# jkworldchampion/Video-Depth-Anything

Measured on AMD Instinct MI355X. Metric: frames/sec at 1x32x518x518 fp16, ViT-L, higher is better.
Workload: dtype f16; 1 GPU; vitl fp16 32-frame clip forward, x=randn(1,32,3,518,518), seeded random weights (BASELINE.json configs[2]); parallelism=independent windows x1, world=1

## Files before the change

include/vda.h:

```cpp
#ifndef VDA_H
#define VDA_H
#include <stddef.h>
#include <stdint.h>

#ifdef __cplusplus
extern "C" {
#endif

typedef void* vda_stream_t;

const char* vda_last_error(void);
int vda_abi_version(void);

enum vda_a_mode {
    VDA_A_DENSE = 0,
    VDA_A_CONV3X3 = 1
};

enum vda_epilogue {
    VDA_EPI_BIAS_F16 = 0,
    VDA_EPI_BIAS_GELU_F16 = 1,
    VDA_EPI_BIAS_RELU_F16 = 2,
    VDA_EPI_SCALE_RES_F32 = 3,
    VDA_EPI_RES_F16 = 4,
// ... 122 lines not shown

int vda_readout_concat_f16(const void* tok, void* out, int frames, int P, int D, vda_stream_t stream);
int vda_readout_concat_f32(const float* tok, float* out, int frames, int P, int D, vda_stream_t stream);

int vda_head_out_f16_f32(const void* in, const float* w, float bias, float* out, int rows, int Cpad, vda_stream_t stream);
int vda_head_out_f32_f32(const float* in, const float* w, float bias, float* out, long long rows, int Cpad, vda_stream_t stream);

int vda_depth_tail_f16(const void* in, const void* w2, const float* b2, const float* w3, float b3, float* out,
                       const void* zero_page, int B, int h, int w, int H, int W, int C, vda_stream_t stream);
int vda_depth_tail_set_variant(int v);
const char* vda_depth_tail_last_kernel(void);

int vda_conv3x3_up2_f16(const void* in, const void* w, const float* bias, void* out, int B, int h, int wd, int C, int N, int ldc,
                        vda_stream_t stream);
int vda_conv3x3_up2_set_variant(int v);
int vda_conv_lds_set_variant(int v);

int vda_normalize_u8_f32(const uint8_t* frames, float* out, int n, int H, int W, vda_stream_t stream);
int vda_gather_normalize_u8_f32(const uint8_t* video, const int32_t* idx, float* out, int n, int n_video, int H, int W,
                                vda_stream_t stream);

int vda_gather_resize_normalize_u8_f32(const uint8_t* video, const int32_t* idx, float* out, int n, int n_video, int H0, int W0,
                                       int H, int W, vda_stream_t stream);

int vda_lsq_scale_shift_f32(const float* pred, const float* target, long long n, double* workspace, int nblk, float* scale_shift,
                            vda_stream_t stream);
int vda_stitch_window_f32(const float* win, const float* scale_shift, float* chunk, float* tail, float* ref1, long long px,
                          const float* wts, vda_stream_t stream);
int vda_affine_clamp_f32(const float* in, const float* scale_shift, float* out, long long n, vda_stream_t stream);
int vda_minmax_accum_f32(const float* x, long long n, float* minmax, vda_stream_t stream);
// ... 94 lines not shown
```

video_depth_anything_amd/_lib.py:

```python
import ctypes as C
import os

_HERE = os.path.dirname(os.path.abspath(__file__))
LIB_PATH = os.environ.get("VDA_LIB_PATH") or os.path.join(_HERE, "libvda_hip.so")

A_DENSE, A_CONV3X3 = 0, 1
(EPI_BIAS_F16, EPI_BIAS_GELU_F16, EPI_BIAS_RELU_F16, EPI_SCALE_RES_F32, EPI_RES_F16, EPI_GEGLU_F16,
 EPI_PATCH_F32, EPI_CONVT_F16, EPI_BIAS_F32, EPI_SCALE_RES_F32_H, EPI_SCALE_RES_SPLIT, EPI_LN_BIAS_F16, EPI_LN_GELU_F16,
 EPI_CONVT_FOLD_F16) = range(14)


class GemmArgs(C.Structure):
    _fields_ = [
        ("A", C.c_void_p), ("W", C.c_void_p), ("bias", C.c_void_p), ("out", C.c_void_p),
        ("res", C.c_void_p), ("res2", C.c_void_p), ("gamma", C.c_void_p), ("pos", C.c_void_p),
        ("zero_page", C.c_void_p),
        ("M", C.c_int32), ("N", C.c_int32), ("K", C.c_int32),
        ("lda", C.c_int32), ("ldc", C.c_int32),
        ("a_mode", C.c_int32), ("epilogue", C.c_int32), ("relu_in", C.c_int32),
        ("cB", C.c_int32), ("cH", C.c_int32), ("cW", C.c_int32), ("cCin", C.c_int32),
        ("cHo", C.c_int32), ("cWo", C.c_int32), ("cStride", C.c_int32),
        ("P", C.c_int32), ("tK", C.c_int32), ("tH", C.c_int32), ("tW", C.c_int32), ("tCout", C.c_int32),
        ("out2", C.c_void_p), ("stats", C.c_void_p), ("sched", C.c_void_p),
        ("stats_ld", C.c_int32), ("tile_rows", C.c_int32),
# ... 31 lines not shown
    "vda_gemm_row_range": (_i, [C.POINTER(GemmArgs), _i, _i, C.POINTER(GemmArgs)]),
    "vda_gemm_last_kernel": (C.c_char_p, []),
    "vda_gemm_plan": (_i, [C.POINTER(GemmArgs), _i, _i, _i, C.POINTER(GemmPlan)]),
    "vda_gemm_launch_name": (_i, [C.POINTER(GemmLaunch), C.c_char_p, _i]),
    "vda_gemm_built": (_i, [_i, _i, _i, _i, _i, _i]),
    "vda_gemm_reload_tuning": (_i, []),
    "vda_layernorm_f32_f16": (_i, [_vp, _vp, _vp, _vp, _f, _i, _i, _i, _i, _vp, _i, _i, _vp]),
    "vda_layernorm_residual_f32_f16": (_i, [_vp, _vp, _vp, _vp, _vp, _vp, _f, _i, _i, _i, _i, _vp]),
    "vda_layernorm_f32_f32": (_i, [_vp, _vp, _vp, _vp, _f, _i, _i, _i, _i, _vp, _i, _i, _vp]),
    "vda_split_stats_f32": (_i, [_vp, _vp, _vp, _vp, _f, _i, _i, _vp]),
    "vda_split_center_stats_f32": (_i, [_vp, _vp, _vp, _vp, _f, _i, _i, _vp]),
    "vda_ln_stats_finalize": (_i, [_vp, _vp, _f, _i, _i, _vp, _vp]),
    "vda_layernorm_split_f16": (_i, [_vp, _vp, _vp, _vp, _vp, _f, _i, _i, _i, _i, _vp]),
    "vda_fold_ln_weight": (_i, [_vp, _vp, _vp, _vp, _vp, _vp, _vp, _i, _i, _vp]),
    "vda_fold_convt_weight": (_i, [_vp, _vp, _vp, _vp, _vp, _i, _i, _i, _i, _i, _vp]),
    "vda_mlp_fused_supported": (_i, [_i, _i]),
    "vda_mlp_permute_w2_f16": (_i, [_vp, _vp, _i, _i, _vp]),
    "vda_mlp_fused_f16": (_i, [_vp, _vp, _vp, _vp, _vp, _vp, _vp, _vp, _vp, _vp, _vp, _i, _i, _i, _i, _vp]),
    "vda_groupnorm_nhwc_f16": (_i, [_vp, _vp, _vp, _vp, _f, _i, _i, _i, _i, _vp, _i, _vp]),
    "vda_groupnorm_nhwc_f32": (_i, [_vp, _vp, _vp, _vp, _f, _i, _i, _i, _i, _vp, _i, _vp]),
    "vda_attention_f16": (_i, [_vp, _vp, _i, _i, _i, _vp]),
    "vda_attention_f32": (_i, [_vp, _vp, _i, _i, _i, _vp]),
    "vda_attention_set_variant": (_i, [_i]),
    "vda_depth_tail_set_variant": (_i, [_i]),
    "vda_depth_tail_last_kernel": (C.c_char_p, []),
    "vda_conv3x3_up2_set_variant": (_i, [_i]),
    "vda_conv_lds_set_variant": (_i, [_i]),
    "vda_temporal_attention_f16": (_i, [_vp, _vp, _i, _i, _i, _i, _vp]),
    "vda_temporal_attention_f32": (_i, [_vp, _vp, _i, _i, _i, _i, _vp]),
    "vda_temporal_attention_set_variant": (_i, [_i]),
# ... 107 lines not shown
```

video_depth_anything_amd/build.py:

```python
import os
import subprocess
import sys
from concurrent.futures import ThreadPoolExecutor

HERE = os.path.dirname(os.path.abspath(__file__))
CSRC = os.path.join(HERE, "csrc")
OBJ = os.path.join(CSRC, "build")
LIB = os.path.join(HERE, "libvda_hip.so")
HIPCC = os.environ.get("HIPCC", "/opt/rocm/bin/hipcc")
FLAGS = ["--offload-arch=gfx950", "-O3", "-std=c++17", "-fPIC", "-ffp-contract=fast", "-Wno-unused-result",
         "-mllvm", "-amdgpu-mfma-vgpr-form"]
PER_FILE = {"stitch.hip": ["-ffp-contract=off"], "eval.hip": ["-ffp-contract=off"], "tae.hip": ["-ffp-contract=off"],
            "resize.hip": ["-ffp-contract=off"], "pointcloud.hip": ["-ffp-contract=off"], "visualize.hip": ["-ffp-contract=off"],
            "losses.hip": ["-ffp-contract=off"], "resize_u8.hip": ["-ffp-contract=off"]}
PER_PREFIX = {"gemm": ["-fno-slp-vectorize"], "attention.hip": ["-fno-slp-vectorize"], "mlp_fused.hip": ["-fno-slp-vectorize"],
              "gemm8p": ["-mllvm", "-amdgpu-atomic-optimizer-strategy=None"]}


def _sources():
    return sorted(f for f in os.listdir(CSRC) if f.endswith(".hip"))


def _deps_mtime():
    hdrs = [os.path.join(CSRC, f) for f in os.listdir(CSRC) if f.endswith(".h")]
    hdrs.append(os.path.join(HERE, "..", "include", "vda.h"))
    return max(os.path.getmtime(h) for h in hdrs)


def _compile(src):
    obj = os.path.join(OBJ, src[:-4] + ".o")
# ... 48 lines not shown
```

video_depth_anything_amd/csrc/host.hip:

```cpp
#include "vda_common.h"
#include <string.h>
#include <exception>
#include <type_traits>
#include <array>
#include <map>
#include <string>
#include <vector>

namespace {

constexpr int PATCH = 14, POS_GRID = 37, KPATCH = 640, GN_GROUPS = 32, TEMPORAL_HEADS = 8;
constexpr float ENC_LN_EPS = 1e-6f, GN_EPS = 1e-6f, TMP_LN_EPS = 1e-5f;

inline int pad64(int c) { return (c + 63) / 64 * 64; }

#define VDA_TRY(expr)            \
    do {                         \
        const int rc_ = (expr);  \
        if (rc_ != 0) return rc_; \
    } while (0)

#define VDA_HIP(expr)                                                      \
    do {                                                                   \
        const hipError_t e_ = (expr);                                      \
// ... 118 lines not shown
    int dyn_sched = 0;
    int ln_fold = VDA_LN_FOLD_DEFAULT;
    int oc1_fused = 1;
    int head_overlap = 0;
    struct Side {
        hipStream_t stream = nullptr;
        hipEvent_t fork = nullptr, join = nullptr, join2 = nullptr;
    };
    std::map<hipStream_t, Side> sides;
    int enc_split = 1;
    std::map<hipStream_t, Side> lanes;
    std::map<hipStream_t, hipEvent_t> tails;
    int head_lanes = 1;
    int convt_fold = 1;
    bool folded[2] = {false, false};
    int mlp_fused = 0;
    volatile int32_t* ovf_host = nullptr;
};

namespace {

using Spec = std::map<std::string, std::vector<int64_t>>;

void build_spec(const vda_config& c, Spec& s) {
    const int64_t D = c.embed_dim, F = c.features;
    const int64_t oc[4] = {c.out_channels[0], c.out_channels[1], c.out_channels[2], c.out_channels[3]};
    auto put = [&](const std::string& k, std::vector<int64_t> v) { s[k] = std::move(v); };
    const std::string p = "pretrained.";
    put(p + "cls_token", {1, 1, D});
    put(p + "pos_embed", {1, POS_GRID * POS_GRID + 1, D});
// ... 225 lines not shown
        VDA_TRY(mat(k + ".w", (size_t)kk * kk * cp * cp, &d));
        hipLaunchKernelGGL((pack_convt_kernel<T>), dim3(grid_for((size_t)kk * kk * cp * cp)), dim3(256), 0, s, raw(n + ".weight"), d, oc[i], oc[i], kk, cp);
        if (vecs) {
            void* bp = nullptr;
            VDA_TRY(dev_alloc(h, (size_t)kk * kk * cp * sizeof(float), &bp));
            h->vec[k + ".b"] = (float*)bp;
            hipLaunchKernelGGL(expand_convt_bias_kernel, dim3((kk * kk * cp + 255) / 256), dim3(256), 0, s, raw(n + ".bias"), (float*)bp, oc[i], kk * kk, cp);
        }
    }
    VDA_TRY(conv("resize3.w", hd + "resize_layers.3.weight", oc[3], oc[3], ocp[3], ocp[3]));
    VDA_TRY(vecp("resize3.b", hd + "resize_layers.3.bias", oc[3], ocp[3]));
    const std::string sc = hd + "scratch.";
    for (int i = 0; i < 4; ++i)
        VDA_TRY(conv("rn" + std::to_string(i + 1) + ".w", sc + "layer" + std::to_string(i + 1) + "_rn.weight", Fe, oc[i], Fe, ocp[i]));
    if constexpr (std::is_same<T, h16>::value) {
        for (int i = 0; i < 2; ++i) {
            const int kk = i == 0 ? 4 : 2;
            const std::string k = "rn" + std::to_string(i + 1) + ".fold";
            T* d = nullptr;
            VDA_TRY(mat(k + ".w", (size_t)kk * kk * Fe * 9 * ocp[i], &d));
            void* bp = nullptr;
            VDA_TRY(dev_alloc(h, (size_t)kk * kk * 9 * Fe * sizeof(float), &bp));
            h->vec[k + ".b"] = (float*)bp;
            VDA_TRY(vda_fold_convt_weight(raw(hd + "resize_layers." + std::to_string(i) + ".weight"), raw(hd + "resize_layers." + std::to_string(i) + ".bias"),
                                          raw(sc + "layer" + std::to_string(i + 1) + "_rn.weight"), d, (float*)bp, kk, oc[i], oc[i], Fe, ocp[i], s));
        }
    }
    for (int i = 1; i <= 4; ++i) {
        const std::string r = sc + "refinenet" + std::to_string(i) + ".", k = "ref" + std::to_string(i) + ".";
        VDA_TRY(lin(k + "out.w", r + "out_conv.weight", Fe, Fe, Fe, Fe));
// ... 262 lines not shown
        const std::string k = "ref" + std::to_string(i) + ".rcu" + std::to_string(u) + ".";
        return conv3x3(x, k + "c1.w", y, B, H, Wd, Fe, Fe, VDA_EPI_BIAS_RELU_F16, 1, V(k + "c1.b"), true);
    }
    int rcu(int i, int u, const void* x, void* out, int B, int H, int Wd, int Fe, const void* res2 = nullptr, const void* y1 = nullptr) {
        const std::string k = "ref" + std::to_string(i) + ".rcu" + std::to_string(u) + ".";
        const void* y = y1;
        if (y1 == nullptr) {
            void* t = act(sp + "rcu_y", (size_t)B * H * Wd * Fe);
            VDA_TRY(rcu_conv1(i, u, x, t, B, H, Wd, Fe));
            y = t;
        }
        VDA_TRY(conv3x3(y, k + "c2.w", out, B, H, Wd, Fe, Fe, VDA_EPI_RES_F16, 1, V(k + "c2.b"), false, x, res2));
        return 0;
    }
    int fusion(int i, const void* x0, const void* x1, int B, int H, int Wd, int Ho, int Wo, int Fe, const std::string& tag, void** result,
               bool upsample = true, const void* y1 = nullptr) {
        const size_t rows = (size_t)B * H * Wd;
        const void* sm = x0;
        if (x1 != nullptr) {
            void* t = act(sp + "fus_s", rows * Fe);
            VDA_TRY(rcu(i, 1, x1, t, B, H, Wd, Fe, x0, y1));
            sm = t;
        }
        void* r = act(sp + "fus_r", rows * Fe);
        VDA_TRY(rcu(i, 2, sm, r, B, H, Wd, Fe));
        void* c = act(upsample ? sp + "fus_c" : tag, rows * Fe);
        const std::string k = "ref" + std::to_string(i) + ".out.";
        VDA_TRY(dense(r, W(k + "w"), c, VDA_EPI_BIAS_F16, (int)rows, Fe, Fe, V(k + "b")));
        if (!upsample) {
            *result = c;
            return 0;
        }
        void* out = act(tag, (size_t)B * Ho * Wo * Fe);
        VDA_TRY(bilinear(c, out, B, H, Wd, Ho, Wo, Fe));
        *result = out;
        return 0;
    }

    int forward(const float* x, float* depth, int B, int T, int H, int Wd) {
        const vda_config& c = h->cfg;
        const int BT = B * T, ph = H / PATCH, pw = Wd / PATCH;
// ... 302 lines not shown
        void* l4 = act("l4", (size_t)BT * h4 * w4 * ocp[3]);
        VDA_TRY(conv3x3(t3, "resize3.w", l4, BT, ph, pw, ocp[3], ocp[3], VDA_EPI_BIAS_F16, 2, V("resize3.b")));
        void* l4t = nullptr;
        VDA_TRY(temporal(1, l4, B, T, h4 * w4, ocp[3], "l4t", &l4t));
        void* l4r = act("l4r", (size_t)BT * h4 * w4 * Fe);
        VDA_TRY(conv3x3(l4t, "rn4.w", l4r, BT, h4, w4, ocp[3], Fe, VDA_EPI_BIAS_F16, 1, nullptr));
        void *p4 = nullptr, *p4t = nullptr, *p3 = nullptr, *p3t = nullptr, *p2 = nullptr, *p1 = nullptr;
        VDA_TRY(fusion(4, l4r, nullptr, BT, h4, w4, ph, pw, Fe, "p4", &p4));
        VDA_TRY(temporal(2, p4, B, T, P, Fe, "p4t", &p4t));
        if (hlanes) VDA_HIP(hipStreamWaitEvent(s, lane->join, 0));
        VDA_TRY(fusion(3, p4t, l3r, BT, ph, pw, h2, w2, Fe, "p3", &p3, true, hlanes ? y1[3] : nullptr));
        VDA_TRY(temporal(3, p3, B, T, h2 * w2, Fe, "p3t", &p3t));
        if (hlanes) VDA_HIP(hipStreamWaitEvent(s, lane->join2, 0));
        VDA_TRY(fusion(2, p3t, l2r, BT, h2, w2, h1, w1, Fe, "p2", &p2, true, hlanes ? y1[2] : nullptr));
        const bool up_fused = prec == VDA_PREC_F16 && h->oc1_fused != 0 && Fhp <= 128 && Fe % 16 == 0;
        VDA_TRY(fusion(1, p2, l1r, BT, h1, w1, 2 * h1, 2 * w1, Fe, up_fused ? "p1c" : "p1", &p1, !up_fused, hlanes ? y1[1] : nullptr));
        const int hh = 2 * h1, ww = 2 * w1;
        void* o1 = act("o1", (size_t)BT * hh * ww * Fhp);
        if (up_fused) {
            if (!dry) VDA_TRY(vda_conv3x3_up2_f16(p1, W("oc1.w"), V("oc1.b"), o1, BT, h1, w1, Fe, Fhp, Fhp, s));
        } else
            VDA_TRY(conv3x3(p1, "oc1.w", o1, BT, hh, ww, Fe, Fhp, VDA_EPI_BIAS_F16, 1, V("oc1.b")));
        if (prec == VDA_PREC_F16) {
            if (!dry) VDA_TRY(vda_depth_tail_f16(o1, W("oc2.w"), V("oc2.b"), V("oc3.w"), h->oc3_bias, depth, h->zero_page, BT, hh, ww, H, Wd, Fhp, s));
        } else {
            void* up = act("tail_up", (size_t)BT * H * Wd * Fhp);
            VDA_TRY(bilinear(o1, up, BT, hh, ww, H, Wd, Fhp));
            void* c2 = act("tail_c2", (size_t)BT * H * Wd * 32);
            VDA_TRY(conv3x3(up, "oc2.w", c2, BT, H, Wd, Fhp, 32, VDA_EPI_BIAS_RELU_F16, 1, V("oc2.b")));
            if (!dry) VDA_TRY(vda_head_out_f32_f32((const float*)c2, V("oc3.w"), h->oc3_bias, depth, (long long)BT * H * Wd, 32, s));
        }
        if (fold && !dry) {
            hipLaunchKernelGGL(poison_on_overflow_kernel, dim3(256), dim3(256), 0, s, (const int*)ovf, depth, (long long)BT * H * Wd, (volatile int*)h->ovf_host);
            VDA_LAUNCH_CHECK();
        }
// ... 34 lines not shown
    VDA_REQUIRE(T <= h->cfg.num_frames, "vda_forward: T=%d exceeds temporal_max_len=%d", T, h->cfg.num_frames);
    VDA_REQUIRE((long long)B * T * ((H / PATCH) * (W / PATCH) + 1) * 4 * h->cfg.embed_dim < (1ll << 31), "vda_forward: clip too large for 32-bit row offsets (B*T*tokens*4*embed_dim)");
    return 0;
}

int head_lanes_default() {
    static const int v = getenv("VDA_HEAD_LANES") ? atoi(getenv("VDA_HEAD_LANES")) : 1;
    return v != 0;
}

int convt_fold_default() {
    static const int v = getenv("VDA_CONVT_FOLD") ? atoi(getenv("VDA_CONVT_FOLD")) : 1;
    return v != 0;
}

int enc_split_default() {
    static const int v = getenv("VDA_ENC_SPLIT") ? atoi(getenv("VDA_ENC_SPLIT")) : 1;
    return v != 0;
}

}

extern "C" int vda_create(const vda_config* cfg, vda_model** out) {
    VDA_REQUIRE(cfg && out, "vda_create: null argument");
    VDA_REQUIRE(cfg->embed_dim > 0 && cfg->embed_dim % 64 == 0 && cfg->num_heads > 0 && cfg->embed_dim == cfg->num_heads * 64,
                "vda_create: embed_dim=%d must be num_heads=%d x 64 (the attention kernels are built for head dim 64)", cfg->embed_dim, cfg->num_heads);
    VDA_REQUIRE(cfg->depth > 0 && cfg->features > 0 && cfg->features % 64 == 0, "vda_create: depth=%d features=%d (features must be a multiple of 64)", cfg->depth, cfg->features);
    VDA_REQUIRE(cfg->num_frames > 0 && cfg->num_frames <= 32, "vda_create: num_frames=%d must be in 1..32", cfg->num_frames);
    VDA_REQUIRE((cfg->use_clstoken | cfg->use_bn | cfg->pe_rope) >> 1 == 0, "vda_create: use_clstoken / use_bn / pe_rope are 0 or 1");
    for (int i = 0; i < 4; ++i) {
// ... 18 lines not shown
        vda_set_error("vda_create: device allocation failed");
        return 2;
    }
    void* ring = nullptr;
    if (hipHostMalloc(&ring, 64, hipHostMallocDefault) != hipSuccess) {
        for (void* p : h->owned) (void)hipFree(p);
        delete h;
        vda_set_error("vda_create: pinned host allocation failed");
        return 2;
    }
    memset(ring, 0, 64);
    h->ovf_host = (volatile int32_t*)ring;
    h->enc_split = enc_split_default();
    h->head_lanes = head_lanes_default();
    h->convt_fold = convt_fold_default();
    *out = h;
    return 0;
}

extern "C" int vda_destroy(vda_model* h) {
    if (h == nullptr) return 0;
    if (h->ovf_host) (void)hipHostFree((void*)h->ovf_host);
    for (auto& kv : h->tails)
        if (kv.second) (void)hipEventDestroy(kv.second);
    for (auto* m : {&h->sides, &h->lanes})
        for (auto& kv : *m) {
            if (kv.second.fork) (void)hipEventDestroy(kv.second.fork);
            if (kv.second.join) (void)hipEventDestroy(kv.second.join);
            if (kv.second.join2) (void)hipEventDestroy(kv.second.join2);
            if (kv.second.stream) (void)hipStreamDestroy(kv.second.stream);
// ... 146 lines not shown

static int vda_debug_copy_impl(vda_model* h, const char* name, void* dst, int64_t bytes, vda_stream_t stream) {
    VDA_REQUIRE(h && name && dst, "vda_debug_copy: null argument");
    auto it = h->layouts.find(h->last_key);
    VDA_REQUIRE(it != h->layouts.end() && h->ws, "vda_debug_copy: no forward has run");
    auto b = it->second.bufs.find(name);
    VDA_REQUIRE(b != it->second.bufs.end(), "vda_debug_copy: no buffer named %s", name);
    VDA_REQUIRE(bytes > 0 && (size_t)bytes <= b->second.second, "vda_debug_copy: %s holds %lld bytes", name, (long long)b->second.second);
    const int lvl = strcmp(name, "l1") == 0 ? 0 : strcmp(name, "l2") == 0 ? 1 : -1;
    if (lvl >= 0 && h->last_key[4] == VDA_PREC_F16 && h->folded[lvl]) {
        VDA_TRY(require_device(h, "vda_debug_copy"));
        Run r{h, VDA_PREC_F16, false, &it->second, (hipStream_t)stream, (size_t)2};
        const int BT = h->last_key[0] * h->last_key[1], ph = h->last_key[2] / PATCH, pw = h->last_key[3] / PATCH;
        VDA_TRY(r.convt(r.act(lvl == 0 ? "t0" : "t1", 0), lvl, r.act(name, 0), BT, ph, pw, h->ocp[lvl]));
    }
    VDA_HIP(hipMemcpyAsync(dst, (char*)h->ws + b->second.first, (size_t)bytes, hipMemcpyDeviceToDevice, (hipStream_t)stream));
    return 0;
}

extern "C" int vda_set_option(vda_model* h, const char* name, int value) {
    VDA_REQUIRE(h && name, "vda_set_option: null argument");
    if (strcmp(name, "residual_in_ln") == 0) {
        h->residual_in_ln = value;
        h->layouts.clear();
        return 0;
    }
    if (strcmp(name, "profile_min_gflop") == 0) {
        h->prof.min_flops = 1e9 * value;
        return 0;
    }
// ... 10 lines not shown
    if (strcmp(name, "head_overlap") == 0) {
        h->head_overlap = value != 0;
        return 0;
    }
    if (strcmp(name, "enc_split") == 0) {
        h->enc_split = value < 0 ? enc_split_default() : value != 0;
        h->layouts.clear();
        return 0;
    }
    if (strcmp(name, "head_lanes") == 0) {
        h->head_lanes = value < 0 ? head_lanes_default() : value != 0;
        return 0;
    }
    if (strcmp(name, "convt_fold") == 0) {
        h->convt_fold = value < 0 ? convt_fold_default() : value != 0;
        return 0;
    }
    if (strcmp(name, "mlp_fused") == 0) {
        h->mlp_fused = value != 0;
        h->layouts.clear();
        return 0;
    }
    if (strcmp(name, "oc1_fused") == 0) {
        h->oc1_fused = value;
        h->layouts.clear();
        return 0;
    }
    vda_set_error("vda_set_option: unknown option %s", name);
    return 1;
}
// ... 111 lines not shown
```

video_depth_anything_amd/engine.py:

```python
import ctypes
import os
from typing import Dict, List

import torch

from . import _lib, ops
from .config import ENC_LN_EPS, GN_EPS, GN_GROUPS, PATCH, POS_GRID, TEMPORAL_HEADS, TMP_LN_EPS, ModelConfig
from .weights import check_state_dict, temporal_channels

F16, F32 = torch.float16, torch.float32
KPATCH = 640


def _pad(c):
    return ops.pad_to(c, 64)


class Engine:
    def __init__(self, cfg: ModelConfig, device="cuda"):
        if not torch.cuda.is_available():
            raise RuntimeError("video_depth_anything_amd needs an MI355X (HIP device); there is no CPU path")
        self.cfg = cfg
        self.device = torch.device(device)
        self.w: Dict[str, torch.Tensor] = {}
        self.act = F16
        self._packs: Dict[torch.dtype, Dict[str, torch.Tensor]] = {}
        self._buf: Dict[tuple, torch.Tensor] = {}
        self._pos_cache: Dict[tuple, torch.Tensor] = {}
        self.loaded = False
        self.residual_in_ln = False
        self.convt_fold = int(os.environ.get("VDA_CONVT_FOLD", "1")) != 0

    def load_state_dict(self, sd, strict=True):
        check_state_dict(self.cfg, sd, strict)
        self._sd = sd
        self._packs.clear()
        self._pos_cache.clear()
        with torch.cuda.device(self.device):
            self._pos_embed_dev = sd["pretrained.pos_embed"].detach().to(self.device, F32).reshape(-1, self.cfg.embed_dim).contiguous()
            self.w = self._pack(F16)
        self.loaded = True

    def _pack(self, dt):
        if dt in self._packs:
            return self._packs[dt]
        cfg, sd = self.cfg, self._sd
# ... 50 lines not shown
        for i in range(4):
            w[f"rn{i + 1}.w"] = conv(f"{sc}layer{i + 1}_rn.weight", Fe, ocp[i])
        if dt == F16:
            for i in (0, 1):
                w[f"rn{i + 1}.fold.w"], w[f"rn{i + 1}.fold.b"] = ops.fold_convt_weight(
                    f32(f"{h}resize_layers.{i}.weight"), f32(f"{h}resize_layers.{i}.bias"), f32(f"{sc}layer{i + 1}_rn.weight"), ocp[i])
        for i in (1, 2, 3, 4):
            r = f"{sc}refinenet{i}."
            w[f"ref{i}.out.w"], w[f"ref{i}.out.b"] = lin(r + "out_conv.weight"), f32(r + "out_conv.bias")
            for u in (1, 2):
                for c in (1, 2):
                    w[f"ref{i}.rcu{u}.c{c}.w"] = conv(f"{r}resConfUnit{u}.conv{c}.weight")
                    w[f"ref{i}.rcu{u}.c{c}.b"] = f32(f"{r}resConfUnit{u}.conv{c}.bias")
        w["oc1.w"] = conv(sc + "output_conv1.weight", Fhp, Fe)
        w["oc1.b"] = padvec(sc + "output_conv1.bias", Fhp)
        w["oc2.w"] = conv(sc + "output_conv2.0.weight", 32, Fhp)
        w["oc2.b"] = f32(sc + "output_conv2.0.bias")
        w["oc3.w"] = f32(sc + "output_conv2.2.weight").reshape(-1)
        self.oc3_bias = float(sd[sc + "output_conv2.2.bias"].reshape(-1)[0])
        for m, Cc in enumerate(temporal_channels(cfg)):
            t = f"{h}motion_modules.{m}.temporal_transformer."
            k = f"tm{m}."
            w[k + "gn.w"], w[k + "gn.b"] = f32(t + "norm.weight"), f32(t + "norm.bias")
            w[k + "in.w"], w[k + "in.b"] = lin(t + "proj_in.weight"), f32(t + "proj_in.bias")
            w[k + "out.w"], w[k + "out.b"] = lin(t + "proj_out.weight"), f32(t + "proj_out.bias")
            tb = t + "transformer_blocks.0."
            for a in (0, 1):
                ab = f"{tb}attention_blocks.{a}."
                qkv = torch.cat([sd[ab + "to_q.weight"], sd[ab + "to_k.weight"], sd[ab + "to_v.weight"]], dim=0)
                w[f"{k}a{a}.qkv.w"] = ops.pack_linear(qkv.detach().to(dv, F32), dtype=dt)
# ... 79 lines not shown
        ops.layernorm(hs, n, w[k + "ffln.w"], w[k + "ffln.b"], TMP_LN_EPS, rows, Cc)
        gg = self.buf("tm_gg", (rows, 4 * Cc), self.act)
        ops.gemm(n, w[k + "ff1.w"], gg, _lib.EPI_GEGLU_F16, M=rows, N=8 * Cc, K=Cc, ldc=4 * Cc, bias=w[k + "ff1.b"])
        hh = self.buf("tm_hh", (rows, Cc), self.act)
        ops.gemm(gg, w[k + "ff2.w"], hh, _lib.EPI_SCALE_RES_F32_H, M=rows, N=Cc, K=4 * Cc, bias=w[k + "ff2.b"], res=hs)
        out = self.buf(tag, (rows, Cc), self.act)
        ops.gemm(hh, w[k + "out.w"], out, _lib.EPI_RES_F16, M=rows, N=Cc, K=Cc, bias=w[k + "out.b"], res=x)
        return out

    def rcu(self, i, u, x, out, B, H, W, Fe, res2=None):
        w = self.w
        y = self.buf("rcu_y", (B * H * W, Fe), self.act)
        self.conv3x3(x, f"ref{i}.rcu{u}.c1.w", y, B, H, W, Fe, Fe, _lib.EPI_BIAS_RELU_F16, bias=w[f"ref{i}.rcu{u}.c1.b"], relu_in=True)
        self.conv3x3(y, f"ref{i}.rcu{u}.c2.w", out, B, H, W, Fe, Fe, _lib.EPI_RES_F16, bias=w[f"ref{i}.rcu{u}.c2.b"], res=x, res2=res2)

    def fusion(self, i, x0, x1, B, H, W, Ho, Wo, Fe, tag, upsample=True):
        w = self.w
        rows = B * H * W
        s = x0
        if x1 is not None:
            s = self.buf("fus_s", (rows, Fe), self.act)
            self.rcu(i, 1, x1, s, B, H, W, Fe, res2=x0)
        r = self.buf("fus_r", (rows, Fe), self.act)
        self.rcu(i, 2, s, r, B, H, W, Fe)
        c = self.buf("fus_c" if upsample else tag, (rows, Fe), self.act)
        ops.gemm(r, w[f"ref{i}.out.w"], c, _lib.EPI_BIAS_F16, M=rows, N=Fe, K=Fe, bias=w[f"ref{i}.out.b"])
        if not upsample:
            return c
        out = self.buf(tag, (B * Ho * Wo, Fe), self.act)
        ops.bilinear_nhwc(c, out, B, H, W, Ho, Wo, Fe)
        return out

    @torch.no_grad()
    def forward(self, x, taps_out: List[torch.Tensor] = None, stages: dict = None, fp32: bool = False):
        if not self.loaded:
            raise RuntimeError("load_state_dict() first")
        with torch.cuda.device(self.device):
            return self._forward(x, taps_out, stages, fp32)

    def _forward(self, x, taps_out, stages, fp32):
# ... 115 lines not shown
        if fold1:
            convt_fold(1, t1, l2r)
        else:
            self.conv3x3(l2, "rn2.w", l2r, BT, h2, w2, ocp[1], Fe, _lib.EPI_BIAS_F16)
        l3r = self.buf("l3r", (BT * P, Fe), self.act)
        self.conv3x3(l3, "rn3.w", l3r, BT, ph, pw, ocp[2], Fe, _lib.EPI_BIAS_F16)
        l4r = self.buf("l4r", (BT * h4 * w4, Fe), self.act)
        self.conv3x3(l4, "rn4.w", l4r, BT, h4, w4, ocp[3], Fe, _lib.EPI_BIAS_F16)

        p4 = self.fusion(4, l4r, None, BT, h4, w4, ph, pw, Fe, "p4")
        p4 = self.temporal(2, p4, B, T, P, Fe, "p4t")
        p3 = self.fusion(3, p4, l3r, BT, ph, pw, h2, w2, Fe, "p3")
        p3 = self.temporal(3, p3, B, T, h2 * w2, Fe, "p3t")
        p2 = self.fusion(2, p3, l2r, BT, h2, w2, h1, w1, Fe, "p2")
        up_fused = not fp32 and Fhp <= 128
        p1 = self.fusion(1, p2, l1r, BT, h1, w1, 2 * h1, 2 * w1, Fe, "p1c" if up_fused else "p1", upsample=not up_fused)

        hh, ww = 2 * h1, 2 * w1
        o1 = self.buf("o1", (BT * hh * ww, Fhp), self.act)
        if up_fused:
            ops.conv3x3_up2(p1, w["oc1.w"], w["oc1.b"], o1, BT, h1, w1, Fe, Fhp, Fhp)
        else:
            self.conv3x3(p1, "oc1.w", o1, BT, hh, ww, Fe, Fhp, _lib.EPI_BIAS_F16, bias=w["oc1.b"])
        depth = torch.empty(B, T, H, W, dtype=F32, device=self.device)
        if not fp32:
            ops.depth_tail(o1, w["oc2.w"], w["oc2.b"], w["oc3.w"], self.oc3_bias, depth, BT, hh, ww, H, W, Fhp)
        else:
            up = self.buf("tail_up", (BT * H * W, Fhp), F32)
            ops.bilinear_nhwc(o1, up, BT, hh, ww, H, W, Fhp)
            c2 = self.buf("tail_c2", (BT * H * W, 32), F32)
            self.conv3x3(up, "oc2.w", c2, BT, H, W, Fhp, 32, _lib.EPI_BIAS_RELU_F16, bias=w["oc2.b"])
            ops.head_out(c2, w["oc3.w"], self.oc3_bias, depth, BT * H * W, 32)
        if stages is not None:
            if fold0:
                convt(0, t0, l1)
            if fold1:
                convt(1, t1, l2)
            stages.update(layer_1=(l1, h1, w1, ocp[0]), layer_2=(l2, h2, w2, ocp[1]), layer_3=(l3, ph, pw, ocp[2]),
                          layer_4=(l4, h4, w4, ocp[3]), path_4=(p4, ph, pw, Fe), path_3=(p3, h2, w2, Fe),
                          path_2=(p2, h1, w1, Fe))
            stages.update(path_1_half=(p1, h1, w1, Fe)) if up_fused else stages.update(path_1=(p1, hh, ww, Fe))
        return depth
```

video_depth_anything_amd/ops.py:

```python
import ctypes as C

import torch

import os
import sys

from . import _lib
from ._lib import GemmArgs, lib
from ._lib import check as _check

_TRACE = os.environ.get("VDA_TRACE_SYNC") == "1"


def check(rc, what=""):
    _check(rc, what)
    if _TRACE:
        sys.stderr.write(f"[vda] {what} ...")
        sys.stderr.flush()
        torch.cuda.synchronize()
        sys.stderr.write(" ok\n")
        sys.stderr.flush()

F16, F32 = torch.float16, torch.float32

# ... 111 lines not shown


def fold_convt_weight(wt, bt, wr, cin_pad=None):
    _req(wt, F32, "wt"), _req(bt, F32, "bt"), _req(wr, F32, "wr")
    Ci, Cm, k, _ = wt.shape
    Co = wr.shape[0]
    if wr.shape[1] != Cm or bt.numel() != Cm or tuple(wr.shape[2:]) != (3, 3) or wt.shape[3] != k:
        raise ValueError("fold_convt_weight: wt [Ci,Cm,k,k], bt [Cm], wr [Co,Cm,3,3]")
    cin_pad = Ci if cin_pad is None else cin_pad
    wf = torch.empty(k * k * Co, 9 * cin_pad, dtype=F16, device=wt.device)
    bc = torch.empty(k * k, 9, Co, dtype=F32, device=wt.device)
    check(lib.vda_fold_convt_weight(_p(wt), _p(bt), _p(wr), _p(wf), _p(bc), k, Ci, Cm, Co, cin_pad, _stream(wt)), "vda_fold_convt_weight")
    return wf, bc


def mlp_permute_w2(w2, w2p, D, hidden):
    _req(w2, F16, "w2"), _req(w2p, F16, "w2p")
    check(lib.vda_mlp_permute_w2_f16(_p(w2), _p(w2p), D, hidden, _stream(w2)), "vda_mlp_permute_w2_f16")


def mlp_fused(hi_in, stats, w1, c1, c2, w2p, b2, gamma, hi, lo, part, M, D, hidden, stats_ld=None):
    for t, n in ((hi_in, "hi_in"), (w1, "w1"), (w2p, "w2p"), (hi, "hi"), (lo, "lo")):
        _req(t, F16, n)
    for t, n in ((stats, "stats"), (c1, "c1"), (c2, "c2"), (b2, "b2"), (gamma, "gamma"), (part, "part")):
        _req(t, F32, n)
    check(lib.vda_mlp_fused_f16(_p(hi_in), _p(stats), _p(w1), _p(c1), _p(c2), _p(w2p), _p(b2), _p(gamma), _p(hi), _p(lo), _p(part), M, D, hidden,
                                M if stats_ld is None else stats_ld, _stream(hi)), "vda_mlp_fused_f16")


def layernorm(x, out, w, b, eps, rows, D, group=0, skip=0, pe=None, pe_rows_per_step=0, pe_steps=0):
# ... 447 lines not shown
```

Measured before the change: 649.2 frames/s.

## Fold refinenet1 out_conv into output_conv1 and combine taps after upsampling

```diff
diff --git a/include/vda.h b/include/vda.h
--- a/include/vda.h
+++ b/include/vda.h
@@ -160,6 +160,12 @@
 int vda_conv3x3_up2_f16(const void* in, const void* w, const float* bias, void* out, int B, int h, int wd, int C, int N, int ldc,
                         vda_stream_t stream);
 int vda_conv3x3_up2_set_variant(int v);
+
+int vda_fold_oc1_weight(const float* W1, const float* Wo, const float* bo, void* Wz, float* bz, int Fh, int Fe, int Fhp, int ldz, vda_stream_t stream);
+int vda_oc1_mix_combine_f16(const void* z, const float* bias, void* out, int B, int h, int w, int Fhp, int ldz, vda_stream_t stream);
+int vda_oc1_mix_ldz(int Fhp);
+int vda_oc1_mix_frames(void);
+int vda_oc1_mix_default(int features);
 int vda_conv_lds_set_variant(int v);
 
 int vda_normalize_u8_f32(const uint8_t* frames, float* out, int n, int H, int W, vda_stream_t stream);
diff --git a/video_depth_anything_amd/_lib.py b/video_depth_anything_amd/_lib.py
--- a/video_depth_anything_amd/_lib.py
+++ b/video_depth_anything_amd/_lib.py
@@ -69,6 +69,11 @@
     "vda_layernorm_split_f16": (_i, [_vp, _vp, _vp, _vp, _vp, _f, _i, _i, _i, _i, _vp]),
     "vda_fold_ln_weight": (_i, [_vp, _vp, _vp, _vp, _vp, _vp, _vp, _i, _i, _vp]),
     "vda_fold_convt_weight": (_i, [_vp, _vp, _vp, _vp, _vp, _i, _i, _i, _i, _i, _vp]),
+    "vda_fold_oc1_weight": (_i, [_vp, _vp, _vp, _vp, _vp, _i, _i, _i, _i, _vp]),
+    "vda_oc1_mix_combine_f16": (_i, [_vp, _vp, _vp, _i, _i, _i, _i, _i, _vp]),
+    "vda_oc1_mix_ldz": (_i, [_i]),
+    "vda_oc1_mix_frames": (_i, []),
+    "vda_oc1_mix_default": (_i, [_i]),
     "vda_mlp_fused_supported": (_i, [_i, _i]),
     "vda_mlp_permute_w2_f16": (_i, [_vp, _vp, _i, _i, _vp]),
     "vda_mlp_fused_f16": (_i, [_vp, _vp, _vp, _vp, _vp, _vp, _vp, _vp, _vp, _vp, _vp, _i, _i, _i, _i, _vp]),
diff --git a/video_depth_anything_amd/build.py b/video_depth_anything_amd/build.py
--- a/video_depth_anything_amd/build.py
+++ b/video_depth_anything_amd/build.py
@@ -14,6 +14,7 @@
             "resize.hip": ["-ffp-contract=off"], "pointcloud.hip": ["-ffp-contract=off"], "visualize.hip": ["-ffp-contract=off"],
             "losses.hip": ["-ffp-contract=off"], "resize_u8.hip": ["-ffp-contract=off"]}
 PER_PREFIX = {"gemm": ["-fno-slp-vectorize"], "attention.hip": ["-fno-slp-vectorize"], "mlp_fused.hip": ["-fno-slp-vectorize"],
+              "oc1_mix.hip": ["-fno-slp-vectorize"],
               "gemm8p": ["-mllvm", "-amdgpu-atomic-optimizer-strategy=None"]}
 
 
diff --git a/video_depth_anything_amd/csrc/host.hip b/video_depth_anything_amd/csrc/host.hip
--- a/video_depth_anything_amd/csrc/host.hip
+++ b/video_depth_anything_amd/csrc/host.hip
@@ -1,5 +1,6 @@
 #include "vda_common.h"
 #include <string.h>
+#include <algorithm>
 #include <exception>
 #include <type_traits>
 #include <array>
@@ -156,6 +157,9 @@
     int head_lanes = 1;
     int convt_fold = 1;
     bool folded[2] = {false, false};
+    int oc1_mix = 0;
+    int oc1_mix_chunk = 0;
+    bool mixed = false;
     int mlp_fused = 0;
     volatile int32_t* ovf_host = nullptr;
 };
@@ -411,6 +415,16 @@
     for (int i = 0; i < 4; ++i)
         VDA_TRY(conv("rn" + std::to_string(i + 1) + ".w", sc + "layer" + std::to_string(i + 1) + "_rn.weight", Fe, oc[i], Fe, ocp[i]));
     if constexpr (std::is_same<T, h16>::value) {
+        {
+            T* d = nullptr;
+            const int ldz = vda_oc1_mix_ldz(Fhp);
+            VDA_TRY(mat("oc1.mix.w", (size_t)ldz * Fe, &d));
+            void* bp = nullptr;
+            VDA_TRY(dev_alloc(h, (size_t)ldz * sizeof(float), &bp));
+            h->vec["oc1.mix.b"] = (float*)bp;
+            VDA_TRY(vda_fold_oc1_weight(raw(sc + "output_conv1.weight"), raw(sc + "refinenet1.out_conv.weight"), raw(sc + "refinenet1.out_conv.bias"), d, (float*)bp,
+                                        Fh, Fe, Fhp, ldz, s));
+        }
         for (int i = 0; i < 2; ++i) {
             const int kk = i == 0 ? 4 : 2;
             const std::string k = "rn" + std::to_string(i + 1) + ".fold";
@@ -703,7 +717,7 @@
         return 0;
     }
     int fusion(int i, const void* x0, const void* x1, int B, int H, int Wd, int Ho, int Wo, int Fe, const std::string& tag, void** result,
-               bool upsample = true, const void* y1 = nullptr) {
+               bool upsample = true, const void* y1 = nullptr, bool no_out = false) {
         const size_t rows = (size_t)B * H * Wd;
         const void* sm = x0;
         if (x1 != nullptr) {
@@ -714,6 +728,10 @@
         void* r = act(sp + "fus_r", rows * Fe);
         VDA_TRY(rcu(i, 2, sm, r, B, H, Wd, Fe));
         void* c = act(upsample ? sp + "fus_c" : tag, rows * Fe);
+        if (no_out) {
+            *result = r;
+            return 0;
+        }
         const std::string k = "ref" + std::to_string(i) + ".out.";
         VDA_TRY(dense(r, W(k + "w"), c, VDA_EPI_BIAS_F16, (int)rows, Fe, Fe, V(k + "b")));
         if (!upsample) {
@@ -1046,11 +1064,24 @@
         if (hlanes) VDA_HIP(hipStreamWaitEvent(s, lane->join2, 0));
         VDA_TRY(fusion(2, p3t, l2r, BT, h2, w2, h1, w1, Fe, "p2", &p2, true, hlanes ? y1[2] : nullptr));
         const bool up_fused = prec == VDA_PREC_F16 && h->oc1_fused != 0 && Fhp <= 128 && Fe % 16 == 0;
-        VDA_TRY(fusion(1, p2, l1r, BT, h1, w1, 2 * h1, 2 * w1, Fe, up_fused ? "p1c" : "p1", &p1, !up_fused, hlanes ? y1[1] : nullptr));
+        const int mixF = std::min(BT, h->oc1_mix_chunk > 0 ? h->oc1_mix_chunk : vda_oc1_mix_frames());
+        const int ldz = vda_oc1_mix_ldz(Fhp);
+        const bool mix_fits = (double)mixF * h1 * w1 * ldz < 2147483647.0;
+        const bool mix = up_fused && !dry && h->oc1_mix != 0 && mix_fits;
+        if (!dry) h->mixed = mix;
+        VDA_TRY(fusion(1, p2, l1r, BT, h1, w1, 2 * h1, 2 * w1, Fe, up_fused ? "p1c" : "p1", &p1, !up_fused, hlanes ? y1[1] : nullptr, mix));
         const int hh = 2 * h1, ww = 2 * w1;
         void* o1 = act("o1", (size_t)BT * hh * ww * Fhp);
+        if (up_fused && mix_fits && (mix || dry)) {
+            void* z = act("oc1_z", (size_t)mixF * h1 * w1 * ldz);
+            for (int f0 = 0; f0 < BT; f0 += mixF) {
+                const int nf = std::min(mixF, BT - f0);
+                VDA_TRY(dense((const h16*)p1 + (size_t)f0 * h1 * w1 * Fe, W("oc1.mix.w"), z, VDA_EPI_BIAS_F16, nf * h1 * w1, ldz, Fe, V("oc1.mix.b")));
+                if (!dry) VDA_TRY(vda_oc1_mix_combine_f16(z, V("oc1.b"), (h16*)o1 + (size_t)f0 * hh * ww * Fhp, nf, h1, w1, Fhp, ldz, s));
+            }
+        }
         if (up_fused) {
-            if (!dry) VDA_TRY(vda_conv3x3_up2_f16(p1, W("oc1.w"), V("oc1.b"), o1, BT, h1, w1, Fe, Fhp, Fhp, s));
+            if (!dry && !mix) VDA_TRY(vda_conv3x3_up2_f16(p1, W("oc1.w"), V("oc1.b"), o1, BT, h1, w1, Fe, Fhp, Fhp, s));
         } else
             VDA_TRY(conv3x3(p1, "oc1.w", o1, BT, hh, ww, Fe, Fhp, VDA_EPI_BIAS_F16, 1, V("oc1.b")));
         if (prec == VDA_PREC_F16) {
@@ -1115,6 +1146,8 @@
     return v != 0;
 }
 
+int oc1_mix_default(const vda_model* h) { return vda_oc1_mix_default(h->cfg.features); }
+
 int enc_split_default() {
     static const int v = getenv("VDA_ENC_SPLIT") ? atoi(getenv("VDA_ENC_SPLIT")) : 1;
     return v != 0;
@@ -1163,6 +1196,7 @@
     h->enc_split = enc_split_default();
     h->head_lanes = head_lanes_default();
     h->convt_fold = convt_fold_default();
+    h->oc1_mix = oc1_mix_default(h);
     *out = h;
     return 0;
 }
@@ -1339,6 +1373,16 @@
         const int BT = h->last_key[0] * h->last_key[1], ph = h->last_key[2] / PATCH, pw = h->last_key[3] / PATCH;
         VDA_TRY(r.convt(r.act(lvl == 0 ? "t0" : "t1", 0), lvl, r.act(name, 0), BT, ph, pw, h->ocp[lvl]));
     }
+    if (strcmp(name, "p1c") == 0 && h->last_key[4] == VDA_PREC_F16 && h->mixed) {
+        VDA_TRY(require_device(h, "vda_debug_copy"));
+        Run r{h, VDA_PREC_F16, false, &it->second, (hipStream_t)stream, (size_t)2};
+        const int BT = h->last_key[0] * h->last_key[1], ph = h->last_key[2] / PATCH, pw = h->last_key[3] / PATCH, Fe = h->cfg.features;
+        const int keep = h->dyn_sched;
+        h->dyn_sched = 0;
+        const int rc = r.dense(r.act("fus_r", 0), r.W("ref1.out.w"), r.act("p1c", 0), VDA_EPI_BIAS_F16, BT * 16 * ph * pw, Fe, Fe, r.V("ref1.out.b"));
+        h->dyn_sched = keep;
+        VDA_TRY(rc);
+    }
     VDA_HIP(hipMemcpyAsync(dst, (char*)h->ws + b->second.first, (size_t)bytes, hipMemcpyDeviceToDevice, (hipStream_t)stream));
     return 0;
 }
@@ -1379,6 +1423,15 @@
     }
     if (strcmp(name, "convt_fold") == 0) {
         h->convt_fold = value < 0 ? convt_fold_default() : value != 0;
+        return 0;
+    }
+    if (strcmp(name, "oc1_mix") == 0) {
+        h->oc1_mix = value < 0 ? oc1_mix_default(h) : value != 0;
+        return 0;
+    }
+    if (strcmp(name, "oc1_mix_chunk") == 0) {
+        h->oc1_mix_chunk = value;
+        h->layouts.clear();
         return 0;
     }
     if (strcmp(name, "mlp_fused") == 0) {
diff --git a/video_depth_anything_amd/csrc/oc1_mix.hip b/video_depth_anything_amd/csrc/oc1_mix.hip
--- /dev/null
+++ b/video_depth_anything_amd/csrc/oc1_mix.hip
@@ -0,0 +1,178 @@
+#include "vda_common.h"
+
+namespace {
+
+constexpr int NT = 256;
+constexpr int TY = 16;
+#ifndef VDA_OC1_MIX_FRAMES
+#define VDA_OC1_MIX_FRAMES 32
+#endif
+#ifndef VDA_OC1_MIX_MIN_FEATURES
+#define VDA_OC1_MIX_MIN_FEATURES 256
+#endif
+
+__global__ void __launch_bounds__(256) fold_oc1_weight_kernel(const float* __restrict__ W1, const float* __restrict__ Wo, h16* __restrict__ Wz, int Fh, int Fe,
+                                                              int Fhp, int ldz) {
+    const long long total = (long long)ldz * Fe;
+    for (long long i = (long long)blockIdx.x * 256 + threadIdx.x; i < total; i += (long long)gridDim.x * 256) {
+        const int ci = (int)(i % Fe);
+        const int co = (int)((i / Fe) % Fhp);
+        const int tap = (int)(i / ((long long)Fe * Fhp));
+        float acc = 0.f;
+        if (co < Fh && tap < 9) {
+            const float* w1 = W1 + (size_t)co * Fe * 9 + tap;
+            for (int cm = 0; cm < Fe; ++cm) acc = fmaf(w1[(size_t)cm * 9], Wo[(size_t)cm * Fe + ci], acc);
+        }
+        Wz[i] = (h16)acc;
+    }
+}
+
+__global__ void __launch_bounds__(256) fold_oc1_bias_kernel(const float* __restrict__ W1, const float* __restrict__ bo, float* __restrict__ bz, int Fh, int Fe,
+                                                            int Fhp, int ldz) {
+    const int i = blockIdx.x * 256 + threadIdx.x;
+    if (i >= ldz) return;
+    const int co = i % Fhp, tap = i / Fhp;
+    float acc = 0.f;
+    if (co < Fh && tap < 9) {
+        const float* w1 = W1 + (size_t)co * Fe * 9 + tap;
+        for (int cm = 0; cm < Fe; ++cm) acc = fmaf(w1[(size_t)cm * 9], bo[cm], acc);
+    }
+    bz[i] = acc;
+}
+
+__global__ void __launch_bounds__(NT) __attribute__((amdgpu_waves_per_eu(4, 8)))
+oc1_mix_combine_kernel(const h16* __restrict__ z, const float* __restrict__ bias, h16* __restrict__ out, int h, int w, int Fhp, int N9, int CL, int TX) {
+    const int tid = threadIdx.x;
+    const int xi = tid / CL, c8 = (tid - xi * CL) * 8;
+    const int H = 2 * h, W = 2 * w;
+    const int X = blockIdx.x * TX + xi, y0 = blockIdx.y * TY, b = blockIdx.z;
+    if (xi >= TX || X >= W) return;
+    const float ys = H > 1 ? (float)(h - 1) / (float)(H - 1) : 0.f, xs = W > 1 ? (float)(w - 1) / (float)(W - 1) : 0.f;
+    int offa[3], offb[3];
+    float wa[3], wb[3];
+#pragma unroll
+    for (int kx = 0; kx < 3; ++kx) {
+        const int qx = X + kx - 1;
+        const bool ok = (unsigned)qx < (unsigned)W;
+        const float sx = xs * (float)min(max(qx, 0), W - 1);
+        const int xa = min((int)sx, w - 1), xb = min(xa + 1, w - 1);
+        const float fx = sx - (float)xa;
+        wa[kx] = ok ? 1.f - fx : 0.f;
+        wb[kx] = ok ? fx : 0.f;
+        offa[kx] = xa * N9 + kx * Fhp + c8;
+        offb[kx] = xb * N9 + kx * Fhp + c8;
+    }
+    const h16* const zf = z + (size_t)b * h * w * N9;
+    auto fetch = [&](int ky, int sy, h16x8 (&L)[6]) {
+        const h16* const row = zf + (size_t)sy * w * N9 + ky * 3 * Fhp;
+#pragma unroll
+        for (int kx = 0; kx < 3; ++kx) {
+            L[2 * kx] = *reinterpret_cast<const h16x8*>(row + offa[kx]);
+            L[2 * kx + 1] = *reinterpret_cast<const h16x8*>(row + offb[kx]);
+        }
+    };
+    auto hsum = [&](const h16x8 (&L)[6], float (&S)[8]) {
+#pragma unroll
+        for (int e = 0; e < 8; ++e) {
+            float a = wa[0] * (float)L[0][e];
+            a = fmaf(wb[0], (float)L[1][e], a);
+            a = fmaf(wa[1], (float)L[2][e], a);
+            a = fmaf(wb[1], (float)L[3][e], a);
+            a = fmaf(wa[2], (float)L[4][e], a);
+            S[e] = fmaf(wb[2], (float)L[5][e], a);
+        }
+    };
+    auto coord = [&](int qy, int& ya, float& fy) {
+        const float sy = ys * (float)qy;
+        ya = __builtin_amdgcn_readfirstlane(min((int)sy, h - 1));
+        fy = sy - (float)ya;
+    };
+    float SA[3][8], SB[3][8];
+    int cur[3];
+#pragma unroll
+    for (int ky = 0; ky < 3; ++ky) {
+        h16x8 L[2][6];
+        float fy;
+        coord(min(max(y0 + ky - 1, 0), H - 1), cur[ky], fy);
+        fetch(ky, cur[ky], L[0]);
+        fetch(ky, min(cur[ky] + 1, h - 1), L[1]);
+        hsum(L[0], SA[ky]);
+        hsum(L[1], SB[ky]);
+#pragma unroll
+        for (int e = 0; e < 8; ++e) asm volatile("" : "+v"(SA[ky][e]), "+v"(SB[ky][e]));
+        __builtin_amdgcn_sched_barrier(0);
+    }
+    float bv[8];
+#pragma unroll
+    for (int e = 0; e < 8; ++e) bv[e] = bias ? bias[c8 + e] : 0.f;
+    const int y1 = min(y0 + TY, H);
+    h16* op = out + (((size_t)b * H + y0) * W + X) * Fhp + c8;
+    for (int Y = y0; Y < y1; ++Y, op += (size_t)W * Fhp) {
+        float acc[8];
+#pragma unroll
+        for (int e = 0; e < 8; ++e) acc[e] = bv[e];
+#pragma unroll
+        for (int ky = 0; ky < 3; ++ky) {
+            const int qy = Y + ky - 1;
+            if ((unsigned)qy >= (unsigned)H) continue;
+            int ya;
+            float fy;
+            coord(qy, ya, fy);
+            if (ya != cur[ky]) {
+                h16x8 L[6];
+                fetch(ky, min(ya + 1, h - 1), L);
+#pragma unroll
+                for (int e = 0; e < 8; ++e) SA[ky][e] = SB[ky][e];
+                hsum(L, SB[ky]);
+                cur[ky] = ya;
+            }
+            const float uy = 1.f - fy;
+#pragma unroll
+            for (int e = 0; e < 8; ++e) acc[e] = fmaf(fy, SB[ky][e], fmaf(uy, SA[ky][e], acc[e]));
+        }
+        h16x8 o;
+#pragma unroll
+        for (int e = 0; e < 8; ++e) o[e] = (h16)acc[e];
+        *reinterpret_cast<h16x8*>(op) = o;
+    }
+}
+
+}
+
+extern "C" int vda_oc1_mix_frames(void) { return VDA_OC1_MIX_FRAMES; }
+
+extern "C" int vda_oc1_mix_default(int features) {
+    static const int env = getenv("VDA_OC1_MIX") ? atoi(getenv("VDA_OC1_MIX")) : -1;
+    return env >= 0 ? env != 0 : features >= VDA_OC1_MIX_MIN_FEATURES;
+}
+
+extern "C" int vda_oc1_mix_ldz(int Fhp) {
+    const int n = 9 * Fhp, p = (n + 255) / 256 * 256;
+    return (p - n) * 8 <= n ? p : n;
+}
+
+extern "C" int vda_fold_oc1_weight(const float* W1, const float* Wo, const float* bo, void* Wz, float* bz, int Fh, int Fe, int Fhp, int ldz, vda_stream_t stream) {
+    VDA_REQUIRE(W1 && Wo && bo && Wz && bz, "vda_fold_oc1_weight: null argument");
+    VDA_REQUIRE(Fh > 0 && Fe > 0 && Fhp >= Fh && Fhp % 8 == 0 && ldz >= 9 * Fhp && ldz % 8 == 0, "vda_fold_oc1_weight: bad geometry Fh=%d Fe=%d Fhp=%d ldz=%d", Fh, Fe, Fhp, ldz);
+    VDA_REQUIRE((long long)ldz * Fe < (1ll << 31), "vda_fold_oc1_weight: composed weight too large");
+    const long long blocks = ((long long)ldz * Fe + 255) / 256;
+    hipLaunchKernelGGL(fold_oc1_weight_kernel, dim3((unsigned)(blocks < 65536 ? blocks : 65536)), dim3(256), 0, (hipStream_t)stream, W1, Wo, (h16*)Wz, Fh, Fe, Fhp, ldz);
+    VDA_LAUNCH_CHECK();
+    hipLaunchKernelGGL(fold_oc1_bias_kernel, dim3((ldz + 255) / 256), dim3(256), 0, (hipStream_t)stream, W1, bo, bz, Fh, Fe, Fhp, ldz);
+    VDA_LAUNCH_CHECK();
+    return 0;
+}
+
+extern "C" int vda_oc1_mix_combine_f16(const void* z, const float* bias, void* out, int B, int h, int w, int Fhp, int ldz, vda_stream_t stream) {
+    VDA_REQUIRE(z && out, "vda_oc1_mix_combine: null pointer");
+    VDA_REQUIRE(B > 0 && B <= 65535 && h > 0 && w > 0 && Fhp > 0 && Fhp % 8 == 0 && Fhp <= 8 * NT && ldz >= 9 * Fhp && ldz % 8 == 0,
+                "vda_oc1_mix_combine: bad geometry B=%d h=%d w=%d Fhp=%d ldz=%d (multiples of 8, ldz >= 9 Fhp)", B, h, w, Fhp, ldz);
+    VDA_REQUIRE(((uintptr_t)z & 15) == 0 && ((uintptr_t)out & 15) == 0 && ((uintptr_t)bias & 3) == 0, "vda_oc1_mix_combine: alignment (16 bytes)");
+    VDA_REQUIRE((double)h * w * ldz < 2147483647.0 && (double)B * 4 * h * w < 2147483647.0, "vda_oc1_mix_combine: frame exceeds 32-bit element offsets");
+    const int CL = Fhp / 8, TX = NT / CL;
+    const int gx = (2 * w + TX - 1) / TX, gy = (2 * h + TY - 1) / TY;
+    VDA_REQUIRE(gy <= 65535, "vda_oc1_mix_combine: too many row strips");
+    hipLaunchKernelGGL(oc1_mix_combine_kernel, dim3(gx, gy, B), dim3(NT), 0, (hipStream_t)stream, (const h16*)z, bias, (h16*)out, h, w, Fhp, ldz, CL, TX);
+    VDA_LAUNCH_CHECK();
+    return 0;
+}
diff --git a/video_depth_anything_amd/engine.py b/video_depth_anything_amd/engine.py
--- a/video_depth_anything_amd/engine.py
+++ b/video_depth_anything_amd/engine.py
@@ -30,6 +30,8 @@
         self.loaded = False
         self.residual_in_ln = False
         self.convt_fold = int(os.environ.get("VDA_CONVT_FOLD", "1")) != 0
+        self.oc1_mix = _lib.lib.vda_oc1_mix_default(cfg.features) != 0
+        self.oc1_mix_chunk = _lib.lib.vda_oc1_mix_frames()
 
     def load_state_dict(self, sd, strict=True):
         check_state_dict(self.cfg, sd, strict)
@@ -110,6 +112,9 @@
                     w[f"ref{i}.rcu{u}.c{c}.b"] = f32(f"{r}resConfUnit{u}.conv{c}.bias")
         w["oc1.w"] = conv(sc + "output_conv1.weight", Fhp, Fe)
         w["oc1.b"] = padvec(sc + "output_conv1.bias", Fhp)
+        if dt == F16:
+            w["oc1.mix.w"], w["oc1.mix.b"] = ops.fold_oc1_weight(
+                f32(sc + "output_conv1.weight"), f32(sc + "refinenet1.out_conv.weight"), f32(sc + "refinenet1.out_conv.bias"), Fhp)
         w["oc2.w"] = conv(sc + "output_conv2.0.weight", 32, Fhp)
         w["oc2.b"] = f32(sc + "output_conv2.0.bias")
         w["oc3.w"] = f32(sc + "output_conv2.2.weight").reshape(-1)
@@ -219,7 +224,7 @@
         self.conv3x3(x, f"ref{i}.rcu{u}.c1.w", y, B, H, W, Fe, Fe, _lib.EPI_BIAS_RELU_F16, bias=w[f"ref{i}.rcu{u}.c1.b"], relu_in=True)
         self.conv3x3(y, f"ref{i}.rcu{u}.c2.w", out, B, H, W, Fe, Fe, _lib.EPI_RES_F16, bias=w[f"ref{i}.rcu{u}.c2.b"], res=x, res2=res2)
 
-    def fusion(self, i, x0, x1, B, H, W, Ho, Wo, Fe, tag, upsample=True):
+    def fusion(self, i, x0, x1, B, H, W, Ho, Wo, Fe, tag, upsample=True, no_out=False):
         w = self.w
         rows = B * H * W
         s = x0
@@ -229,6 +234,8 @@
         r = self.buf("fus_r", (rows, Fe), self.act)
         self.rcu(i, 2, s, r, B, H, W, Fe)
         c = self.buf("fus_c" if upsample else tag, (rows, Fe), self.act)
+        if no_out:
+            return r
         ops.gemm(r, w[f"ref{i}.out.w"], c, _lib.EPI_BIAS_F16, M=rows, N=Fe, K=Fe, bias=w[f"ref{i}.out.b"])
         if not upsample:
             return c
@@ -374,11 +381,20 @@
         p3 = self.temporal(3, p3, B, T, h2 * w2, Fe, "p3t")
         p2 = self.fusion(2, p3, l2r, BT, h2, w2, h1, w1, Fe, "p2")
         up_fused = not fp32 and Fhp <= 128
-        p1 = self.fusion(1, p2, l1r, BT, h1, w1, 2 * h1, 2 * w1, Fe, "p1c" if up_fused else "p1", upsample=not up_fused)
+        mixF = min(BT, self.oc1_mix_chunk)
+        ldz = _lib.lib.vda_oc1_mix_ldz(Fhp)
+        mix = up_fused and self.oc1_mix and mixF * h1 * w1 * ldz < (1 << 31) - 1
+        p1 = self.fusion(1, p2, l1r, BT, h1, w1, 2 * h1, 2 * w1, Fe, "p1c" if up_fused else "p1", upsample=not up_fused, no_out=mix)
 
         hh, ww = 2 * h1, 2 * w1
         o1 = self.buf("o1", (BT * hh * ww, Fhp), self.act)
-        if up_fused:
+        if mix:
+            z = self.buf("oc1_z", (mixF * h1 * w1, ldz), F16)
+            for f0 in range(0, BT, mixF):
+                nf = min(mixF, BT - f0)
+                ops.gemm(p1[f0 * h1 * w1:(f0 + nf) * h1 * w1], w["oc1.mix.w"], z, _lib.EPI_BIAS_F16, M=nf * h1 * w1, N=ldz, K=Fe, bias=w["oc1.mix.b"])
+                ops.oc1_mix_combine(z, w["oc1.b"], o1[f0 * hh * ww:(f0 + nf) * hh * ww], nf, h1, w1, Fhp, ldz)
+        elif up_fused:
             ops.conv3x3_up2(p1, w["oc1.w"], w["oc1.b"], o1, BT, h1, w1, Fe, Fhp, Fhp)
         else:
             self.conv3x3(p1, "oc1.w", o1, BT, hh, ww, Fe, Fhp, _lib.EPI_BIAS_F16, bias=w["oc1.b"])
@@ -399,5 +415,8 @@
             stages.update(layer_1=(l1, h1, w1, ocp[0]), layer_2=(l2, h2, w2, ocp[1]), layer_3=(l3, ph, pw, ocp[2]),
                           layer_4=(l4, h4, w4, ocp[3]), path_4=(p4, ph, pw, Fe), path_3=(p3, h2, w2, Fe),
                           path_2=(p2, h1, w1, Fe))
+            if mix:
+                r1, p1 = p1, self.buf("p1c", (BT * h1 * w1, Fe), self.act)
+                ops.gemm(r1, w["ref1.out.w"], p1, _lib.EPI_BIAS_F16, M=BT * h1 * w1, N=Fe, K=Fe, bias=w["ref1.out.b"])
             stages.update(path_1_half=(p1, h1, w1, Fe)) if up_fused else stages.update(path_1=(p1, hh, ww, Fe))
         return depth
diff --git a/video_depth_anything_amd/ops.py b/video_depth_anything_amd/ops.py
--- a/video_depth_anything_amd/ops.py
+++ b/video_depth_anything_amd/ops.py
@@ -149,6 +149,27 @@
     return wf, bc
 
 
+def fold_oc1_weight(w1, wo, bo, cout_pad=None, ldz=None):
+    _req(w1, F32, "w1"), _req(wo, F32, "wo"), _req(bo, F32, "bo")
+    Fh, Fe = w1.shape[0], w1.shape[1]
+    if tuple(w1.shape[2:]) != (3, 3) or wo.numel() != Fe * Fe or bo.numel() != Fe:
+        raise ValueError("fold_oc1_weight: w1 [Fh,Fe,3,3], wo [Fe,Fe(,1,1)], bo [Fe]")
+    Fhp = Fh if cout_pad is None else cout_pad
+    ldz = lib.vda_oc1_mix_ldz(Fhp) if ldz is None else ldz
+    wz = torch.empty(ldz, Fe, dtype=F16, device=w1.device)
+    bz = torch.empty(ldz, dtype=F32, device=w1.device)
+    check(lib.vda_fold_oc1_weight(_p(w1), _p(wo), _p(bo), _p(wz), _p(bz), Fh, Fe, Fhp, ldz, _stream(w1)), "vda_fold_oc1_weight")
+    return wz, bz
+
+
+def oc1_mix_combine(z, bias, out, B, h, w, Fhp, ldz=None):
+    ldz = 9 * Fhp if ldz is None else ldz
+    _req(z, F16, "z"), _req(out, F16, "out"), _req(bias, F32, "bias")
+    if z.numel() < B * h * w * ldz or out.numel() < B * 4 * h * w * Fhp or (bias is not None and bias.numel() < Fhp):
+        raise ValueError("oc1_mix_combine buffers too small")
+    check(lib.vda_oc1_mix_combine_f16(_p(z), _p(bias), _p(out), B, h, w, Fhp, ldz, _stream(z)), "vda_oc1_mix_combine_f16")
+
+
 def mlp_permute_w2(w2, w2p, D, hidden):
     _req(w2, F16, "w2"), _req(w2p, F16, "w2p")
     check(lib.vda_mlp_permute_w2_f16(_p(w2), _p(w2p), D, hidden, _stream(w2)), "vda_mlp_permute_w2_f16")
```

New measurement: 660.2 frames/s, median of 6. 1.02x the previous value.
